# pvangoor/eqvio

Hardware: AMD Instinct MI355X
Metric: EqF vision updates/sec @ N=200 landmarks (higher is better)
Workload: dtype f64; 1 GPU; synthetic 'hover' world, 200 tracked landmarks (state dim 621, 400 measurement rows), InvDepth chart, fast Riccati, IMU 200 Hz / camera 20 Hz (10 observer steps per frame), EuRoC pinhole intrinsics, one independent filter per GPU (replicas); landmarks=200, state_dim=621, parallelism=replicas x1

## Files before the change

eqvio_amd/csrc/eqf_kernels.hpp:

```cpp
#pragma once
#include "eqf_math.hpp"
#include "eqvio_types.h"
#include <hip/hip_runtime.h>

namespace eqf {

struct Common {
    double Mv[9];
    double RTic[9];
    double RTicSx[9];
    double CT[36];
    double vC[3];
    double Ass[441];
    double Bs[252];
};
struct CommonK {
    double lm[66];
    double RA[9];
    double SxRA[9];
    double RAsv[9];
    double G[9];
    double adT[36];
};
constexpr int kObsChunk = 20;
struct RiccatiArgs {
    double dt;
    double Qd[12];
    double Pd[8];
};
struct ObsStep {
    int discrete;
    double dt;
    Pose Tinv;
    V3 omC, vC;
};

__device__ __forceinline__ V3 ld3(const double* base, int stride, int i) { return V3{base[i], base[stride + i], base[2 * stride + i]}; }
__device__ __forceinline__ Qt ldq(const double* base, int stride, int i) { return Qt{base[i], base[stride + i], base[2 * stride + i], base[3 * stride + i]}; }
__device__ __forceinline__ M3 ldm3(const double* p) { return M3{p[0], p[1], p[2], p[3], p[4], p[5], p[6], p[7], p[8]}; }
__device__ __forceinline__ void st_plane9(double* base, int stride, int i, int plane0, const M3& A) {
    base[(plane0 + 0) * stride + i] = A.a00;
    base[(plane0 + 1) * stride + i] = A.a01;
    base[(plane0 + 2) * stride + i] = A.a02;
    base[(plane0 + 3) * stride + i] = A.a10;
    base[(plane0 + 4) * stride + i] = A.a11;
    base[(plane0 + 5) * stride + i] = A.a12;
    base[(plane0 + 6) * stride + i] = A.a20;
    base[(plane0 + 7) * stride + i] = A.a21;
    base[(plane0 + 8) * stride + i] = A.a22;
}

typedef unsigned long long trace_t;
__device__ __forceinline__ void trace_start(trace_t* tr) {
    if (tr && blockIdx.x == 0 && blockIdx.y == 0 && threadIdx.x == 0)
        *tr = wall_clock64();
}
__device__ __forceinline__ void trace_end(trace_t* tr) {
    if (tr && threadIdx.x == 0)
        atomicMax(tr + 1, (trace_t)wall_clock64());
}

__device__ __forceinline__ double fast_rcp(double d) {
    double r = __builtin_amdgcn_rcp(d);
    double e = fma(-d, r, 1.0);
    r = fma(r, e, r);
    e = fma(-d, r, 1.0);
    return fma(r, e, r);
}

__device__ __forceinline__ double fast_rsqrt(double x) {
    double y = __builtin_amdgcn_rsq(x);
    double h = 0.5 * x;
    y = y * fma(-h * y, y, 1.5);
    y = y * fma(-h * y, y, 1.5);
    return y;
}
constexpr int CC_OFF = 3, CC_E2I = 0, CC_I2E = 9, CC_R0 = 18, CC_PLANES = 27;
__device__ __forceinline__ M3 ld_cc(const double* __restrict__ q0, int Ncap, int i, int which) {
    const double* b = q0 + (size_t)(CC_OFF + which) * Ncap + i;
    return M3{b[0], b[Ncap], b[2 * (size_t)Ncap], b[3 * (size_t)Ncap], b[4 * (size_t)Ncap], b[5 * (size_t)Ncap], b[6 * (size_t)Ncap], b[7 * (size_t)Ncap], b[8 * (size_t)Ncap]};
}
__device__ __attribute__((noinline)) void store_chart_constants(double* __restrict__ cc, int Ncap, int i, double px, double py, double pz, M3* r0) {
    const V3 p{px, py, pz};
    st_plane9(cc, Ncap, i, CC_E2I, conv_euc2ind(p));
    st_plane9(cc, Ncap, i, CC_I2E, conv_ind2euc(p));
    const M3 R = ind2euc_r0(p);
    st_plane9(cc, Ncap, i, CC_R0, R);
    if (r0)
        *r0 = R;
}

__host__ __device__ __forceinline__ int al_col(int e) { return e < 3 ? e : (e < 6 ? 12 + (e - 3) : 15 + (e - 6)); }

__device__ __forceinline__ double sensor_Bs_entry(const CommonK& ck, int t) {
    const int r = t / 12, c = t % 12;
    double v = 0.0;
    if (r < 6)
        v = (c == 6 + r) ? 1.0 : 0.0;
    else if (r < 9 && c < 3)
        v = ck.RA[(r - 6) * 3 + c];
    else if (r >= 9 && r < 12 && c < 3)
        v = ck.SxRA[(r - 9) * 3 + c];
    else if (r >= 12 && r < 15 && c < 3)
        v = ck.RAsv[(r - 12) * 3 + c];
    else if (r >= 12 && r < 15 && c >= 3 && c < 6)
        v = ck.RA[(r - 12) * 3 + (c - 3)];
    return v;
}
__device__ __forceinline__ double sensor_Ass_entry(const CommonK& ck, int t) {
    const int r = t / 21, c = t % 21;
    double v = 0.0;
    if (c < 6) {
        if (r >= 6 && r < 9 && c < 3)
            v = -ck.RA[(r - 6) * 3 + c];
        else if (r >= 9 && r < 12 && c < 3)
            v = -ck.SxRA[(r - 9) * 3 + c];
        else if (r >= 12 && r < 15 && c < 3)
            v = -ck.RAsv[(r - 12) * 3 + c];
        else if (r >= 12 && r < 15 && c >= 3)
            v = -ck.RA[(r - 12) * 3 + (c - 3)];
    } else if (r >= 9 && r < 12 && c == r + 3) {
        v = 1.0;
    } else if (r >= 12 && r < 15 && c >= 6 && c < 9) {
        v = ck.G[(r - 12) * 3 + (c - 6)];
    } else if (r >= 15 && c >= 15) {
        v = ck.adT[(r - 15) * 6 + (c - 15)];
    }
    return v;
}
template <int PART>
__device__ __forceinline__ void assemble_landmark(const double* __restrict__ s_cm, int chart, const V3 p0, const Qt q, const double a, const M3& e2i, const M3& i2e,
                                                  double (&al)[45], double (&bl)[9]) {
    constexpr bool P0 = PART < 0 || PART == 0, P1 = PART < 0 || PART == 1, P2 = PART < 0 || PART == 2;
    const M3 Mv = ldm3(s_cm), RTic = ldm3(s_cm + 9), RTicSx = ldm3(s_cm + 18);
    const double* CT = s_cm + 27;
    const V3 vC{s_cm[63], s_cm[64], s_cm[65]};
    const M3 RQ = q_mat(q);
    const M3 Qhat = a * RQ;
    const V3 qh = (1.0 / a) * (transpose(RQ) * p0);
    const bool ind = chart == EQVIO_COORD_INVDEPTH;
    if (P0) {
        M3 Bblk = Qhat * (skew(qh) * RTic + RTicSx);
        M3 A_v = (-1.0) * (Qhat * Mv);
        if (ind) {
            Bblk = e2i * Bblk;
            A_v = e2i * A_v;
        }
        const M3 A_b = (-1.0) * Bblk;
        const double ab[9] = {A_b.a00, A_b.a01, A_b.a02, A_b.a10, A_b.a11, A_b.a12, A_b.a20, A_b.a21, A_b.a22};
        const double av[9] = {A_v.a00, A_v.a01, A_v.a02, A_v.a10, A_v.a11, A_v.a12, A_v.a20, A_v.a21, A_v.a22};
#pragma unroll
        for (int r = 0; r < 3; ++r)
#pragma unroll
            for (int c = 0; c < 3; ++c) {
                al[r * 15 + c] = ab[r * 3 + c];
                al[r * 15 + 3 + c] = av[r * 3 + c];
            }
        bl[0] = Bblk.a00, bl[1] = Bblk.a01, bl[2] = Bblk.a02, bl[3] = Bblk.a10, bl[4] = Bblk.a11, bl[5] = Bblk.a12, bl[6] = Bblk.a20, bl[7] = Bblk.a21, bl[8] = Bblk.a22;
    }
    if (P1) {
        const M3 T0 = skew(p0) * RQ;
        const M3 T1 = (-a) * RQ;
        const double t[3][6] = {{T0.a00, T0.a01, T0.a02, T1.a00, T1.a01, T1.a02},
                                {T0.a10, T0.a11, T0.a12, T1.a10, T1.a11, T1.a12},
                                {T0.a20, T0.a21, T0.a22, T1.a20, T1.a21, T1.a22}};
        double Ac[3][6];
#pragma unroll
        for (int r = 0; r < 3; ++r)
#pragma unroll
            for (int c = 0; c < 6; ++c) {
                double s = 0;
#pragma unroll
                for (int k = 0; k < 6; ++k)
                    s += t[r][k] * CT[k * 6 + c];
                Ac[r][c] = s;
            }
        if (ind) {
            const double e[3][3] = {{e2i.a00, e2i.a01, e2i.a02}, {e2i.a10, e2i.a11, e2i.a12}, {e2i.a20, e2i.a21, e2i.a22}};
            double Ac2[3][6];
#pragma unroll
            for (int r = 0; r < 3; ++r)
#pragma unroll
                for (int c = 0; c < 6; ++c)
                    Ac2[r][c] = e[r][0] * Ac[0][c] + e[r][1] * Ac[1][c] + e[r][2] * Ac[2][c];
#pragma unroll
            for (int r = 0; r < 3; ++r)
#pragma unroll
                for (int c = 0; c < 6; ++c)
                    Ac[r][c] = Ac2[r][c];
        }
#pragma unroll
        for (int r = 0; r < 3; ++r)
#pragma unroll
            for (int c = 0; c < 6; ++c)
                al[r * 15 + 6 + c] = Ac[r][c];
    }
    if (P2) {
        const M3 inner = skew(qh) * skew(vC) - 2.0 * outer(vC, qh) + outer(qh, vC);
        const M3 QhatInv = (1.0 / a) * transpose(RQ);
        M3 A_q = (-1.0 / norm2(qh)) * (Qhat * inner * QhatInv);
        if (ind)
            A_q = e2i * A_q * i2e;
        const double aq[9] = {A_q.a00, A_q.a01, A_q.a02, A_q.a10, A_q.a11, A_q.a12, A_q.a20, A_q.a21, A_q.a22};
#pragma unroll
        for (int r = 0; r < 3; ++r)
#pragma unroll
            for (int c = 0; c < 3; ++c)
                al[r * 15 + 12 + c] = aq[r * 3 + c];
    }
}
__global__ void __launch_bounds__(64) k_assemble_AB(const CommonK ck, int N, int Ncap, int chart, Common* __restrict__ cmdev,
                                                    const double* __restrict__ q0, const double* __restrict__ Qq, const double* __restrict__ Qa,
                                                    double* __restrict__ Al, double* __restrict__ Bl, trace_t* tr) {
    trace_start(tr);
    __shared__ double s_cm[9 + 9 + 9 + 36 + 3];
    for (int t = threadIdx.x; t < 66; t += blockDim.x)
        s_cm[t] = ck.lm[t];
    {
        const int gt = blockIdx.x * blockDim.x + threadIdx.x, gs = gridDim.x * blockDim.x;
        for (int t = gt; t < 252; t += gs)
            cmdev->Bs[t] = sensor_Bs_entry(ck, t);
        for (int t = gt; t < 441; t += gs)
            cmdev->Ass[t] = sensor_Ass_entry(ck, t);
    }
    __syncthreads();
    const int i = blockIdx.x * blockDim.x + threadIdx.x;
    if (i >= N)
        return;
    double al[45], bl[9];
    const bool ind = chart == EQVIO_COORD_INVDEPTH;
    assemble_landmark<-1>(s_cm, chart, ld3(q0, Ncap, i), ldq(Qq, Ncap, i), Qa[i], ind ? ld_cc(q0, Ncap, i, CC_E2I) : M3{}, ind ? ld_cc(q0, Ncap, i, CC_I2E) : M3{}, al, bl);
#pragma unroll
    for (int e = 0; e < 45; ++e)
        Al[e * Ncap + i] = al[e];
#pragma unroll
    for (int e = 0; e < 9; ++e)
        Bl[e * Ncap + i] = bl[e];
}

struct ObsSteps {
    ObsStep s[kObsChunk];
};
__device__ __forceinline__ void observer_chain(const ObsStep* __restrict__ steps, int k, const V3 p0, Qt& q, double& a) {
    double inva = 1.0 / a;
    ObsStep nxt = steps[0];
    for (int s = 0; s < k; ++s) {
        const ObsStep st = nxt;
        nxt = steps[min(s + 1, k - 1)];
        const V3 ph = inva * q_rot(q_inv(q), p0);
        Qt Lq;
        double La, invLa;
        if (st.discrete) {
            const V3 p1 = pose_act(st.Tinv, ph);
            const double nh2 = norm2(ph), n12 = norm2(p1);
            const double r = fast_rsqrt(nh2 * n12);
            const double c = dot(p1, ph) * r;
            if (c < -1.0 + 1e-12) {
                Lq = so3_from_vectors(normalized(p1), normalized(ph));
            } else {
                const V3 ax = r * cross(p1, ph);
                const double t = (1.0 + c) * 2.0;
                const double is = fast_rsqrt(t);
                const Qt L{0.5 * (t * is), ax.x * is, ax.y * is, ax.z * is};
                const double kk = 1.5 - 0.5 * (L.w * L.w + L.x * L.x + L.y * L.y + L.z * L.z);
                Lq = Qt{L.w * kk, L.x * kk, L.y * kk, L.z * kk};
            }
            La = nh2 * r;
            invLa = n12 * r;
        } else {
            const double ip2 = 1.0 / norm2(ph);
            const V3 Wr = st.omC + ip2 * cross(ph, st.vC);
            const double Ws = ip2 * dot(ph, st.vC);
            Lq = so3_exp(st.dt * Wr);
            La = exp(st.dt * Ws);
            invLa = 1.0 / La;
        }
        if (st.discrete) {
            const Qt m{q.w * Lq.w - q.x * Lq.x - q.y * Lq.y - q.z * Lq.z, q.w * Lq.x + q.x * Lq.w + q.y * Lq.z - q.z * Lq.y,
                       q.w * Lq.y + q.y * Lq.w + q.z * Lq.x - q.x * Lq.z, q.w * Lq.z + q.z * Lq.w + q.x * Lq.y - q.y * Lq.x};
            const double km = 1.5 - 0.5 * (m.w * m.w + m.x * m.x + m.y * m.y + m.z * m.z);
            q = Qt{m.w * km, m.x * km, m.y * km, m.z * km};
// ... 1114 lines not shown
            swork[tid] = z;
        }
        __syncthreads();
        const int wr = i0 + tid - m;
        if (tid < 32 && wr >= 0 && wr < rows - 1 - m) {
            double gsum = 0.0;
            for (int c = 0; c < w; ++c)
                gsum = fma(sPI[tid + c * CH_LDP], swork[c], gsum);
            gpart[(size_t)GAMMA_G * ldg + wr] = gsum;
        }
    }
    if (!update)
        return;
    const bool next_diag = (blockIdx.x == 0 && blockIdx.y == 0);
    {
        const double* pj = diag_tile ? sPI : sPJ;
        d4 acc = {0, 0, 0, 0};
#pragma unroll
        for (int st = 0; st < 8; ++st) {
            const int c = 4 * st + lk;
            const double a = sPI[16 * ihU + lr + c * CH_LDP];
            const double b = pj[16 * jhU + lr + c * CH_LDP];
            acc = __builtin_amdgcn_mfma_f64_16x16x4f64(b, a, acc, 0, 0, 0);
        }
        const int i = i0 + 16 * ihU + lr;
#pragma unroll
        for (int q = 0; q < 4; ++q) {
            const int j = j0 + 16 * jhU + lk + 4 * q;
            const double v = zt[q] - acc[q];
            if (i < rows && j < m && (!next_diag || i >= m))
                Z[i + (size_t)j * ldz] = v;
            if (next_diag)
                sPJ[16 * ihU + lr + (16 * jhU + lk + 4 * q) * CH_LDP] = v;
        }
    }
    if (!next_diag)
        return;
    __syncthreads();
    const int w2 = min(32, m - c0);
#pragma unroll
    for (int k = 0; k < 4; ++k) {
        const int c = g + 8 * k;
        if (r >= w2 || c >= w2)
            sPJ[r + c * CH_LDP] = (r == c) ? 1.0 : 0.0;
    }
    __syncthreads();
    ldl_inverse_tile(sPJ, CH_LDP, w2, LinvOut, flags, swork);
}

template <typename TS, bool FUSED, bool SYM = false, bool GH = false>
__global__ void __launch_bounds__(PROP_T) k_propagate_main(int N, int Ncap, int ld, RiccatiArgs ra, const Common* __restrict__ cm,
                                                        const TS* __restrict__ Sig, TS* __restrict__ Sout, const double* __restrict__ Al,
                                                        const double* __restrict__ Bl, int nT, int tpw, const ObsSteps obs, int obs_k,
                                                        const double* __restrict__ q0, double* __restrict__ Qq, double* __restrict__ Qa, int nObs, const StageArgs sg,
                                                        trace_t* tr, const FuseArgs fa, const MeasEval me, const GatherArgs ga_in) {
    GatherArgs ga;
    if constexpr (GH)
        ga = ga_in;
    else {
        ga.n = 0, ga.nprop = N, ga.held = nullptr, ga.st_in = nullptr, ga.st_out = nullptr;
    }
    trace_start(tr);
    const double dt = ra.dt;
    const int b = blockIdx.x;
    const int tid = threadIdx.x;
    constexpr bool sym = SYM;
    constexpr int nStrip = 0;
    int nTiles = sym ? nT * (nT + 1) / 2 : nT * nT;
    if (sym && tpw > 1) {
        nTiles = 0;
        for (int r_ = 0; r_ < nT; ++r_)
            nTiles += (r_ + tpw) / tpw;
    }
    __shared__ double sm[2 * PT * (63 + 36 + 9 + 9) + 63 * PT + 12 * 21 + 8];
    __shared__ double sJ1[PT * (63 + 36 + 9 + 9)];
    if (b > nTiles + nStrip + nObs) {
        for (int t = tid; t < 2 * sg.M; t += PROP_T)
            sg.y_d[t] = sg.y_h[t];
        for (int t = tid; t < sg.M; t += PROP_T)
            sg.idx_d[t] = sg.idx_h[t];
        for (int t = tid; t < 3 * N; t += PROP_T) {
            const int pl = t / N, i = t - pl * N;
            sg.ylm_d[pl * Ncap + i] = sg.ylm_h[pl * Ncap + i];
        }
        return;
    }
    if (b > nTiles + nStrip) {
        const int i = (b - (nTiles + nStrip + 1)) * PROP_T + tid;
        static_assert(sizeof(ObsStep) % 8 == 0 && kObsChunk * sizeof(ObsStep) <= sizeof(sm), "the steps are copied as doubles into the tile buffer");
        if (FUSED) {
            for (int t = tid; t < obs_k * (int)(sizeof(ObsStep) / 8); t += PROP_T)
                sm[t] = reinterpret_cast<const double*>(obs.s)[t];
            __syncthreads();
        }
        const ObsStep* steps_lds = reinterpret_cast<const ObsStep*>(sm);
        if (i < N) {
            if (FUSED) {
                const bool held = i >= ga.nprop;
                const bool synth = held && ga.held != nullptr;
                const int io = held ? i : gather_old(ga, i);
                V3 p0;
                Qt q;
                double a_;
                if (synth) {
                    const double* hp = ga.held + 1 + 3 * (i - ga.nprop);
                    p0 = V3{hp[0], hp[1], hp[2]};
                    q = Qt{1.0, 0.0, 0.0, 0.0};
                    a_ = 1.0;
                } else {
                    p0 = ld3(q0, Ncap, io);
                    q = ldq(Qq, Ncap, io);
                    a_ = Qa[io];
                }
                double yu = 0.0, yv = 0.0;
                int jm = -1;
                if (me.on) {
                    yu = me.ylm[i], yv = me.ylm[Ncap + i];
                    jm = (int)me.ylm[2 * Ncap + i];
                }
                M3 r0_new{};
                if (synth) {
                    double* st = ga.st_out;
                    st[i] = p0.x;
                    st[Ncap + i] = p0.y;
                    st[2 * (size_t)Ncap + i] = p0.z;
                    double* cc = st + (size_t)CC_OFF * Ncap;
                    store_chart_constants(cc, Ncap, i, p0.x, p0.y, p0.z, &r0_new);
                }
                if (!held)
                    observer_chain(steps_lds, obs_k, p0, q, a_);
                fa.Qqo[i] = q.w;
                fa.Qqo[Ncap + i] = q.x;
                fa.Qqo[2 * Ncap + i] = q.y;
                fa.Qqo[3 * Ncap + i] = q.z;
                fa.Qao[i] = a_;
                if (me.on && jm >= 0) {
                    asm volatile("" : "+v"(q.w), "+v"(q.x), "+v"(q.y), "+v"(q.z), "+v"(a_));
                    const MeasOut o = measure_one(fa.chart, me.cam, p0, q, a_, yu, yv, me.star != 0, fa.chart == EQVIO_COORD_INVDEPTH ? (synth ? r0_new : ld_cc(q0, Ncap, io, CC_R0)) : M3{});
#pragma unroll
                    for (int e = 0; e < 6; ++e)
                        me.C[e * me.Mcap + jm] = o.c[e];
                    me.ytil[2 * jm] = o.yt[0];
                    me.ytil[2 * jm + 1] = o.yt[1];
                    me.lmidx_dev[jm] = i;
                }
            } else {
                observer_landmark(obs.s, Ncap, obs_k, i, q0, Qq, Qa, Qq, Qa);
            }
        }
        return;
    }
    __shared__ double sSens[21 * 33];
    __shared__ double sSens1[21 * 33];
    __shared__ double s_cm[66];
    if (FUSED) {
        for (int t = tid; t < 66; t += PROP_T)
            s_cm[t] = fa.ck.lm[t];
        __syncthreads();
    }
    if (b < nTiles) {
        int bi = b % nT, bj0 = b / nT, ntile = 1;
        if (sym && tpw > 1) {
            int base = 0;
            bi = 0;
            for (;;) {
                const int w_ = (bi + tpw) / tpw;
                if (b < base + w_)
                    break;
                base += w_;
                ++bi;
            }
            bj0 = (b - base) * tpw;
            ntile = min(tpw, bi + 1 - bj0);
        } else if (sym) {
            bi = (int)((sqrtf(8.0f * (float)b + 1.0f) - 1.0f) * 0.5f);
            while (bi * (bi + 1) / 2 > b)
                --bi;
            while ((bi + 1) * (bi + 2) / 2 <= b)
                ++bi;
            bj0 = b - bi * (bi + 1) / 2;
        }
        const int nb = sym ? bi + 1 : nT;
        const int Nprop = FUSED ? ga.nprop : N;
        const int Nmem = (FUSED && ga.held) ? Nprop : N;
        const double held_var = (FUSED && ga.held && Nprop < N) ? ga.held[0] : 0.0;
        double* sGi = sm;
        double* sFi = sGi + 63 * PT;
        double* sDi = sFi + 36 * PT;
        double* sBi = sDi + 9 * PT;
        double* sJ0 = sBi + 9 * PT;
        double* sSi = sJ0 + 117 * PT;
        double* sSs = sSi + 63 * PT;
        const int r = tid / (PT * PT), tp = tid % (PT * PT);
        const int ti = tp % PT, tj = tp / PT;
        auto stage = [&](const int it) {
            const bool first = it == 0;
            const int bj = bj0 + it;
            double* sSj = (it & 1) ? sJ1 : sJ0;
            double* sFj = sSj + 63 * PT;
            double* sDj = sFj + 36 * PT;
            double* sBj = sDj + 9 * PT;
            double* sSn = (it & 1) ? sSens1 : sSens;
            for (int t = tid; t < 63 * PT; t += PROP_T) {
                const int e = t / PT, x = t % PT;
                const int i = bi * PT + x, j = bj * PT + x;
                const int kk = e / 3, cc = e % 3;
                if (first)
                    sSi[t] = i < Nmem ? Sig[kk + (size_t)(21 + 3 * (i < Nprop ? gather_old(ga, i) : i) + cc) * ld] : 0.0;
                sSj[t] = j < Nmem ? Sig[kk + (size_t)(21 + 3 * (j < Nprop ? gather_old(ga, j) : j) + cc) * ld] : 0.0;
            }
            if (first && tid < 12 * 21)
                sSs[tid] = Sig[al_col(tid / 21) + (size_t)(tid % 21) * ld];
            const int ncol = bj < 21 ? (21 - bj + nb - 1) / nb : 0;
            for (int t = PROP_T - 1 - tid; t < ncol * 33; t += PROP_T) {
                const int m_ = t / 33, e = t % 33;
                const int c = bj + nb * m_;
                sSn[t] = e < 21 ? (FUSED ? sensor_Ass_entry(fa.ck, c * 21 + e) : cm->Ass[c * 21 + e]) : (FUSED ? sensor_Bs_entry(fa.ck, c * 12 + (e - 21)) : cm->Bs[c * 12 + (e - 21)]);
            }
            if (FUSED) {
                const int part = tid >> 6, lane_ = tid & 63;
                if (part < 3 && lane_ < 2 * PT && (first || lane_ >= PT)) {
                    const bool isj = lane_ >= PT;
                    const int x = lane_ % PT;
                    const int l = (isj ? bj : bi) * PT + x;
                    double* dF = isj ? sFj : sFi;
                    double* dD = isj ? sDj : sDi;
                    double* dB = isj ? sBj : sBi;
                    double al[45], bl[9];
#pragma unroll
                    for (int e = 0; e < 45; ++e)
                        al[e] = 0.0;
#pragma unroll
                    for (int e = 0; e < 9; ++e)
                        bl[e] = 0.0;
                    const bool in = l < Nprop;
                    const bool heldl = l >= Nprop && l < N;
                    const bool ind = fa.chart == EQVIO_COORD_INVDEPTH;
                    const int lc = in ? gather_old(ga, l) : 0;
                    const V3 p0_ = ld3(q0, Ncap, lc);
                    const Qt q_ = ldq(Qq, Ncap, lc);
                    const double a_ = Qa[lc];
                    const M3 e2i = ind ? ld_cc(q0, Ncap, lc, CC_E2I) : M3{};
                    if (part == 0) {
                        if (in)
                            assemble_landmark<0>(s_cm, fa.chart, p0_, q_, a_, e2i, M3{}, al, bl);
#pragma unroll
                        for (int rr = 0; rr < 3; ++rr) {
#pragma unroll
                            for (int c = 0; c < 6; ++c)
                                dF[(rr * 12 + c) * PT + x] = in ? dt * al[rr * 15 + c] : 0.0;
#pragma unroll
                            for (int c = 0; c < 3; ++c)
                                dB[(rr * 3 + c) * PT + x] = bl[rr * 3 + c];
                        }
                    } else if (part == 1) {
                        if (in)
                            assemble_landmark<1>(s_cm, fa.chart, p0_, q_, a_, e2i, M3{}, al, bl);
#pragma unroll
                        for (int rr = 0; rr < 3; ++rr)
#pragma unroll
                            for (int c = 6; c < 12; ++c)
                                dF[(rr * 12 + c) * PT + x] = in ? dt * al[rr * 15 + c] : 0.0;
                    } else {
                        if (in)
                            assemble_landmark<2>(s_cm, fa.chart, p0_, q_, a_, e2i, ind ? ld_cc(q0, Ncap, lc, CC_I2E) : M3{}, al, bl);
#pragma unroll
                        for (int rr = 0; rr < 3; ++rr)
#pragma unroll
                            for (int c = 0; c < 3; ++c)
                                dD[(rr * 3 + c) * PT + x] = in ? dt * al[rr * 15 + 12 + c] + ((rr == c) ? 1.0 : 0.0) : ((heldl && rr == c) ? 1.0 : 0.0);
                    }
                }
            } else {
                for (int t = tid; t < 36 * PT; t += PROP_T) {
                    const int e = t / PT, x = t % PT;
                    const int rr = e / 12, c = e % 12;
                    const int i = bi * PT + x, j = bj * PT + x;
                    if (first)
                        sFi[t] = i < N ? dt * Al[(rr * 15 + c) * Ncap + i] : 0.0;
                    sFj[t] = j < N ? dt * Al[(rr * 15 + c) * Ncap + j] : 0.0;
                }
                for (int t = tid; t < 9 * PT; t += PROP_T) {
                    const int e = t / PT, x = t % PT;
                    const int rr = e / 3, c = e % 3;
                    const int i = bi * PT + x, j = bj * PT + x;
                    const double eye = (rr == c) ? 1.0 : 0.0;
                    if (first) {
                        sDi[t] = i < N ? dt * Al[(rr * 15 + 12 + c) * Ncap + i] + eye : 0.0;
                        sBi[t] = i < N ? Bl[e * Ncap + i] : 0.0;
                    }
                    sDj[t] = j < N ? dt * Al[(rr * 15 + 12 + c) * Ncap + j] + eye : 0.0;
                    sBj[t] = j < N ? Bl[e * Ncap + j] : 0.0;
                }
            }
        };
        stage(0);
        __syncthreads();
        for (int t = tid; t < 63 * PT; t += PROP_T) {
            const int e = t / PT, x = t % PT;
            const int rr = e / 21, k = e % 21;
            double g = 0.0;
#pragma unroll
            for (int q = 0; q < 12; ++q)
                g += sFi[(rr * 12 + q) * PT + x] * sSs[q * 21 + k];
#pragma unroll
            for (int cc = 0; cc < 3; ++cc)
                g += sDi[(rr * 3 + cc) * PT + x] * sSi[(k * 3 + cc) * PT + x];
            sGi[t] = g;
        }
        __syncthreads();
        for (int it = 0; it < ntile; ++it) {
            const int bj = bj0 + it;
            const double* sSj = (it & 1) ? sJ1 : sJ0;
            const double* sFj = sSj + 63 * PT;
            const double* sDj = sFj + 36 * PT;
            const double* sBj = sDj + 9 * PT;
            const double* sSn = (it & 1) ? sSens1 : sSens;
            const int ncol = bj < 21 ? (21 - bj + nb - 1) / nb : 0;
            const int i = bi * PT + ti, j = bj * PT + tj;
            const bool mine = !(i >= N || j >= N || (sym && bi == bj && i < j));
            const int li = 21 + 3 * i, lj = 21 + 3 * j;
            double Sij[3][3];
            if (mine) {
                if (i < Nmem && j < Nmem) {
                    const int lio = 21 + 3 * (i < Nprop ? gather_old(ga, i) : i), ljo = 21 + 3 * (j < Nprop ? gather_old(ga, j) : j);
#pragma unroll
                    for (int k = 0; k < 3; ++k)
#pragma unroll
                        for (int c = 0; c < 3; ++c)
                            Sij[k][c] = Sig[lio + k + (size_t)(ljo + c) * ld];
                } else {
#pragma unroll
                    for (int k = 0; k < 3; ++k)
#pragma unroll
                        for (int c = 0; c < 3; ++c)
                            Sij[k][c] = (i == j && k == c) ? held_var : 0.0;
                }
            }
            if (it + 1 < ntile)
                stage(it + 1);
            {
                for (int t = tid; t < PT * 3 * ncol; t += PROP_T) {
                    const int x = t % PT, rc = t / PT;
                    const int rr = rc % 3, m_ = rc / 3, c = bj + nb * m_;
                    const int ii = bi * PT + x;
                    if (ii < N) {
                        double sacc = 0;
                        for (int k = 0; k < 21; ++k) {
                            const double f = dt * sSn[m_ * 33 + k] + (k == c ? 1.0 : 0.0);
                            sacc += sGi[(rr * 21 + k) * PT + x] * f;
                        }
                        double bq = 0;
#pragma unroll
                        for (int q = 0; q < 3; ++q)
                            bq += sBi[(rr * 3 + q) * PT + x] * ra.Qd[q] * sSn[m_ * 33 + 21 + q];
                        sacc += dt * bq;
                        const int lii = 21 + 3 * ii;
                        Sout[lii + rr + (size_t)c * ld] = sacc;
                        Sout[c + (size_t)(lii + rr) * ld] = sacc;
                    }
                }
            }
            if (mine) {
                double E[3];
#pragma unroll
                for (int c = 0; c < 3; ++c) {
                    double s = 0;
#pragma unroll
                    for (int e = 0; e < 12; ++e)
                        s += sFi[(r * 12 + e) * PT + ti] * sSj[(al_col(e) * 3 + c) * PT + tj];
#pragma unroll
                    for (int k = 0; k < 3; ++k)
                        s += sDi[(r * 3 + k) * PT + ti] * Sij[k][c];
                    E[c] = s;
                }
#pragma unroll
                for (int c = 0; c < 3; ++c) {
                    double s = 0;
#pragma unroll
                    for (int e = 0; e < 12; ++e)
                        s += sGi[(r * 21 + al_col(e)) * PT + ti] * sFj[(c * 12 + e) * PT + tj];
#pragma unroll
                    for (int k = 0; k < 3; ++k)
                        s += E[k] * sDj[(c * 3 + k) * PT + tj];
                    double bq = 0;
#pragma unroll
                    for (int q = 0; q < 3; ++q)
                        bq += sBi[(r * 3 + q) * PT + ti] * ra.Qd[q] * sBj[(c * 3 + q) * PT + tj];
                    s += dt * bq;
                    if (i == j && r == c && i < Nprop)
                        s += dt * ra.Pd[7];
                    Sout[li + r + (size_t)(lj + c) * ld] = s;
                    if (sym && i != j)
                        Sout[lj + c + (size_t)(li + r) * ld] = s;
                }
            }
            if (it + 1 < ntile)
                __syncthreads();
        }
        return;
    }
    {
        if (FUSED && ga.n) {
            const int Np = ga.nprop;
            for (int t = tid; t < (CC_OFF + CC_PLANES) * Np; t += PROP_T) {
                const int pl = t / Np, i = t - pl * Np;
                ga.st_out[(size_t)pl * Ncap + i] = ga.st_in[(size_t)pl * Ncap + gather_old(ga, i)];
            }
        }
        double* sF = sm;
        double* sS = sm + 441;
        double* sT = sm + 882;
        double* sBs = sm + 1323;
        for (int t = tid; t < 441; t += PROP_T) {
            const int r = t / 21, c = t % 21;
            sF[t] = dt * (FUSED ? sensor_Ass_entry(fa.ck, t) : cm->Ass[t]) + (r == c ? 1.0 : 0.0);
            sS[t] = Sig[r + (size_t)c * ld];
        }
        for (int t = tid; t < 252; t += PROP_T)
            sBs[t] = FUSED ? sensor_Bs_entry(fa.ck, t) : cm->Bs[t];
        __syncthreads();
        for (int t = tid; t < 441; t += PROP_T) {
            const int r = t / 21, c = t % 21;
            double s = 0;
            for (int k = 0; k < 21; ++k)
                s += sF[r * 21 + k] * sS[k * 21 + c];
            sT[t] = s;
        }
        __syncthreads();
        for (int t = tid; t < 441; t += PROP_T) {
            const int r = t / 21, c = t % 21;
            double s = 0;
            for (int k = 0; k < 21; ++k)
                s += sT[r * 21 + k] * sF[c * 21 + k];
            double bq = 0;
            for (int q = 0; q < 12; ++q)
                bq += sBs[r * 12 + q] * ra.Qd[q] * sBs[c * 12 + q];
            s += dt * bq;
            if (r == c)
                s += dt * ra.Pd[r / 3];
            Sout[r + (size_t)c * ld] = s;
        }
    }
}


#ifndef EQF_SYRK_UNROLL
#define EQF_SYRK_UNROLL 4
#endif
struct TileRed {
    double v[4];
};
template <bool WITH_GEMV, int NW = 4>
__device__ __forceinline__ TileRed mfma_tile32_splitk(const double* __restrict__ P, int ldp, int i0, int rowsP, const double* __restrict__ Qm, int ldq, int j0,
                                                      int rowsQ, int K, double* __restrict__ sred , const double* __restrict__ zvec = nullptr,
                                                      int ldzv = 0, double* gv_out = nullptr) {
    const int tid = threadIdx.x;
    const int wave = tid >> 6, lane = tid & 63;
    const int lr = lane & 15, lk = lane >> 4;
    const int ia = min(i0 + lr, rowsP - 1), ib = min(i0 + 16 + lr, rowsP - 1);
    const int ja = min(j0 + lr, rowsQ - 1), jb = min(j0 + 16 + lr, rowsQ - 1);
    const double zia = (i0 + lr < rowsP) ? 1.0 : 0.0, zib = (i0 + 16 + lr < rowsP) ? 1.0 : 0.0;
    const double zja = (j0 + lr < rowsQ) ? 1.0 : 0.0, zjb = (j0 + 16 + lr < rowsQ) ? 1.0 : 0.0;
    d4 acc00 = {0, 0, 0, 0}, acc10 = acc00, acc01 = acc00, acc11 = acc00;
    double ga = 0.0, gb = 0.0;
    const int nsteps = (K + 3) >> 2;
#pragma unroll EQF_SYRK_UNROLL
    for (int st = wave; st < nsteps; st += NW) {
        const int kk = 4 * st + lk;
        const int kc = min(kk, K - 1);
        const double zk = kk < K ? 1.0 : 0.0;
        const double pa = P[ia + (size_t)kc * ldp] * (zia * zk);
        const double pb = P[ib + (size_t)kc * ldp] * (zib * zk);
        const double qa = Qm[ja + (size_t)kc * ldq] * zja;
        const double qb = Qm[jb + (size_t)kc * ldq] * zjb;
        if (WITH_GEMV) {
            const double zv = zvec[(size_t)kc * ldzv];
            ga = fma(pa, zv, ga);
            gb = fma(pb, zv, gb);
        }
        acc00 = __builtin_amdgcn_mfma_f64_16x16x4f64(qa, pa, acc00, 0, 0, 0);
        acc10 = __builtin_amdgcn_mfma_f64_16x16x4f64(qa, pb, acc10, 0, 0, 0);
        acc01 = __builtin_amdgcn_mfma_f64_16x16x4f64(qb, pa, acc01, 0, 0, 0);
        acc11 = __builtin_amdgcn_mfma_f64_16x16x4f64(qb, pb, acc11, 0, 0, 0);
    }
    TileRed out;
#pragma unroll
    for (int e = 0; e < 4; ++e)
        out.v[e] = 0.0;
#pragma unroll
    for (int q0 = 0; q0 < NW; q0 += 4) {
        if (q0)
            __syncthreads();
        if (wave >= q0 && wave < q0 + 4) {
            double* mine = sred + (wave - q0) * 1024;
#pragma unroll
            for (int r = 0; r < 4; ++r) {
                const int j = lk + 4 * r;
                mine[lr + 32 * j] = acc00[r];
                mine[16 + lr + 32 * j] = acc10[r];
                mine[lr + 32 * (16 + j)] = acc01[r];
                mine[16 + lr + 32 * (16 + j)] = acc11[r];
            }
        }
        __syncthreads();
#pragma unroll
        for (int e = 0; e < 4; ++e) {
            const int idx = (tid & 31) + 32 * (((tid & 255) >> 5) + 8 * e);
            out.v[e] += (sred[idx] + sred[1024 + idx]) + (sred[2048 + idx] + sred[3072 + idx]);
        }
    }
    if (WITH_GEMV) {
        __syncthreads();
        sred[(wave * 4 + lk) * 32 + lr] = ga;
        sred[(wave * 4 + lk) * 32 + 16 + lr] = gb;
        __syncthreads();
        if (tid < 32) {
            double g = 0.0;
#pragma unroll
            for (int q = 0; q < 4 * NW; ++q)
                g += sred[q * 32 + tid];
            *gv_out = g;
        }
    }
    return out;
}

__global__ void __launch_bounds__(256) k_gamma(int n, int m, int ldz, const double* __restrict__ Wb, double* __restrict__ gamma) {
    __shared__ double sp[256];
    const int r = blockIdx.x * 64 + (threadIdx.x & 63);
    const int seg = threadIdx.x >> 6;
    const double* W = Wb + m;
    const double* z = Wb + m + n;
    double s0 = 0, s1 = 0, s2 = 0, s3 = 0;
    if (r < n) {
        int p = seg;
        for (; p + 12 < m; p += 16) {
            s0 += W[r + (size_t)p * ldz] * z[(size_t)p * ldz];
            s1 += W[r + (size_t)(p + 4) * ldz] * z[(size_t)(p + 4) * ldz];
            s2 += W[r + (size_t)(p + 8) * ldz] * z[(size_t)(p + 8) * ldz];
            s3 += W[r + (size_t)(p + 12) * ldz] * z[(size_t)(p + 12) * ldz];
        }
        for (; p < m; p += 4)
            s0 += W[r + (size_t)p * ldz] * z[(size_t)p * ldz];
    }
    sp[threadIdx.x] = (s0 + s1) + (s2 + s3);
    __syncthreads();
    if (seg == 0 && r < n)
        gamma[r] = (sp[threadIdx.x] + sp[64 + threadIdx.x]) + (sp[128 + threadIdx.x] + sp[192 + threadIdx.x]);
}

constexpr int SYRK_ARITH_TILES = 24;
constexpr int SYRK_NW = 8;
template <typename TS, bool WITH_GAMMA>
__device__ __forceinline__ void syrk_sub_tile(int n, int m, int ld, int ldz, const double* __restrict__ Wb, TS* __restrict__ Sig, double* __restrict__ gamma, const int* __restrict__ spec,
                                              int spec_seq, const int* __restrict__ flags, trace_t* tr, const int* __restrict__ tile_of_block, int stall_seq, int blk, const int* __restrict__ live_cols = nullptr, int nt_arith = 0) {
    if (tr && blk == 0 && threadIdx.x == 0)
        *tr = wall_clock64();
    const int f0 = flags[0], f3 = flags[3];
    const int specv = spec ? *spec : 0;
    __shared__ double sred[1024 * 4];
    int bi, bj;
    if (nt_arith > 0) {
        bi = (int)((sqrtf(8.0f * (float)blk + 1.0f) - 1.0f) * 0.5f);
        while ((bi + 1) * (bi + 2) / 2 <= blk)
            ++bi;
        while (bi * (bi + 1) / 2 > blk)
            --bi;
        bj = blk - bi * (bi + 1) / 2;
    } else {
        const int code = tile_of_block[blk];
        bi = code & 0xffff, bj = code >> 16;
    }
// ... 968 lines not shown
```

Baseline: 11590 updates/s.

## Split propagate tile staging across warps and stage sensor constants in LDS

In the fused covariance propagation kernel, warps 0-2 now issue their landmark-state loads early, while the remaining threads batch-load the Sigma landmark/sensor blocks into registers before writing them to shared memory. The whole CommonK struct is also copied into LDS, and the sensor Ass/Bs entries are read from there with index-based lookups instead of branchy reads from kernel arguments. The goal is to overlap global-load latency with assembly work and cut repeated constant-parameter reads. In exchange the code carries more complex thread-role logic, extra registers for the batched loads, and a changed synchronisation pattern.

```diff
diff --git a/eqvio_amd/csrc/eqf_kernels.hpp b/eqvio_amd/csrc/eqf_kernels.hpp
--- a/eqvio_amd/csrc/eqf_kernels.hpp
+++ b/eqvio_amd/csrc/eqf_kernels.hpp
@@ -127,6 +127,36 @@
         v = ck.adT[(r - 15) * 6 + (c - 15)];
     }
     return v;
+}
+constexpr int CK_RA = 66, CK_G = CK_RA + 27, CK_ADT = CK_G + 9, CK_DOUBLES = CK_ADT + 36;
+static_assert(sizeof(CommonK) == CK_DOUBLES * sizeof(double), "CommonK is read as doubles");
+__device__ __forceinline__ double sensor_Bs_entry_lds(const double* s_ck, int t) {
+    const int r = t / 12, c = t % 12, blk = r / 3;
+    int idx = -1;
+    if (blk >= 2 && blk <= 4 && c < 3)
+        idx = CK_RA + 9 * (blk - 2) + (r - 3 * blk) * 3 + c;
+    else if (blk == 4 && c < 6)
+        idx = CK_RA + (r - 12) * 3 + (c - 3);
+    const double v = s_ck[max(idx, 0)];
+    return idx >= 0 ? v : ((r < 6 && c == 6 + r) ? 1.0 : 0.0);
+}
+__device__ __forceinline__ double sensor_Ass_entry_lds(const double* s_ck, int t) {
+    const int r = t / 21, c = t % 21, blk = r / 3;
+    int idx = -1;
+    bool neg = false;
+    if (c < 6) {
+        neg = true;
+        if (blk >= 2 && blk <= 4 && c < 3)
+            idx = CK_RA + 9 * (blk - 2) + (r - 3 * blk) * 3 + c;
+        else if (blk == 4)
+            idx = CK_RA + (r - 12) * 3 + (c - 3);
+    } else if (blk == 4 && c < 9) {
+        idx = CK_G + (r - 12) * 3 + (c - 6);
+    } else if (r >= 15 && c >= 15) {
+        idx = CK_ADT + (r - 15) * 6 + (c - 15);
+    }
+    const double v = s_ck[max(idx, 0)];
+    return idx >= 0 ? (neg ? -v : v) : ((blk == 3 && c == r + 3) ? 1.0 : 0.0);
 }
 template <int PART>
 __device__ __forceinline__ void assemble_landmark(const double* __restrict__ s_cm, int chart, const V3 p0, const Qt q, const double a, const M3& e2i, const M3& i2e,
@@ -1547,10 +1577,11 @@
     }
     __shared__ double sSens[21 * 33];
     __shared__ double sSens1[21 * 33];
-    __shared__ double s_cm[66];
-    if (FUSED) {
-        for (int t = tid; t < 66; t += PROP_T)
-            s_cm[t] = fa.ck.lm[t];
+    __shared__ double s_ck[CK_DOUBLES];
+    const double* const s_cm = s_ck;
+    if (FUSED && b >= nTiles) {
+        for (int t = tid; t < CK_DOUBLES; t += PROP_T)
+            s_ck[t] = reinterpret_cast<const double*>(&fa.ck)[t];
         __syncthreads();
     }
     if (b < nTiles) {
@@ -1596,28 +1627,113 @@
             double* sDj = sFj + 36 * PT;
             double* sBj = sDj + 9 * PT;
             double* sSn = (it & 1) ? sSens1 : sSens;
-            for (int t = tid; t < 63 * PT; t += PROP_T) {
-                const int e = t / PT, x = t % PT;
-                const int i = bi * PT + x, j = bj * PT + x;
-                const int kk = e / 3, cc = e % 3;
-                if (first)
-                    sSi[t] = i < Nmem ? Sig[kk + (size_t)(21 + 3 * (i < Nprop ? gather_old(ga, i) : i) + cc) * ld] : 0.0;
-                sSj[t] = j < Nmem ? Sig[kk + (size_t)(21 + 3 * (j < Nprop ? gather_old(ga, j) : j) + cc) * ld] : 0.0;
-            }
-            if (first && tid < 12 * 21)
-                sSs[tid] = Sig[al_col(tid / 21) + (size_t)(tid % 21) * ld];
             const int ncol = bj < 21 ? (21 - bj + nb - 1) / nb : 0;
-            for (int t = PROP_T - 1 - tid; t < ncol * 33; t += PROP_T) {
-                const int m_ = t / 33, e = t % 33;
-                const int c = bj + nb * m_;
-                sSn[t] = e < 21 ? (FUSED ? sensor_Ass_entry(fa.ck, c * 21 + e) : cm->Ass[c * 21 + e]) : (FUSED ? sensor_Bs_entry(fa.ck, c * 12 + (e - 21)) : cm->Bs[c * 12 + (e - 21)]);
+            if (!FUSED) {
+                for (int t = tid; t < 63 * PT; t += PROP_T) {
+                    const int e = t / PT, x = t % PT;
+                    const int i = bi * PT + x, j = bj * PT + x;
+                    const int kk = e / 3, cc = e % 3;
+                    if (first)
+                        sSi[t] = i < N ? Sig[kk + (size_t)(21 + 3 * i + cc) * ld] : 0.0;
+                    sSj[t] = j < N ? Sig[kk + (size_t)(21 + 3 * j + cc) * ld] : 0.0;
+                }
+                if (first && tid < 12 * 21)
+                    sSs[tid] = Sig[al_col(tid / 21) + (size_t)(tid % 21) * ld];
+                for (int t = PROP_T - 1 - tid; t < ncol * 33; t += PROP_T) {
+                    const int m_ = t / 33, e = t % 33;
+                    const int c = bj + nb * m_;
+                    sSn[t] = e < 21 ? cm->Ass[c * 21 + e] : cm->Bs[c * 12 + (e - 21)];
+                }
             }
             if (FUSED) {
+                constexpr int NA = 3 * 64, NC = PROP_T - NA, SIJ = 63 * PT, NK = (2 * SIJ + 12 * 21 + NC - 1) / NC;
                 const int part = tid >> 6, lane_ = tid & 63;
-                if (part < 3 && lane_ < 2 * PT && (first || lane_ >= PT)) {
-                    const bool isj = lane_ >= PT;
-                    const int x = lane_ % PT;
-                    const int l = (isj ? bj : bi) * PT + x;
+                const bool assembles = part < 3 && lane_ < 2 * PT && (first || lane_ >= PT);
+                const bool isj = lane_ >= PT;
+                const int x = lane_ % PT;
+                const int l = (isj ? bj : bi) * PT + x;
+                const bool in = l < Nprop;
+                const bool heldl = l >= Nprop && l < N;
+                const bool ind = fa.chart == EQVIO_COORD_INVDEPTH;
+                V3 p0_{};
+                Qt q_{};
+                double a_ = 0.0;
+                M3 e2i{}, i2e{};
+                auto request_state = [&]() {
+                    if (assembles) {
+                        const int lc = in ? gather_old(ga, l) : 0;
+                        p0_ = ld3(q0, Ncap, lc);
+                        q_ = ldq(Qq, Ncap, lc);
+                        a_ = Qa[lc];
+                        if (ind)
+                            e2i = ld_cc(q0, Ncap, lc, CC_E2I);
+                        if (ind && part == 2)
+                            i2e = ld_cc(q0, Ncap, lc, CC_I2E);
+                    }
+                };
+                if (first)
+                    request_state();
+                if (tid >= NA) {
+                    const int u = tid - NA;
+                    constexpr int TOT = 2 * SIJ + 12 * 21;
+                    auto item = [&](const int t, size_t& off, bool& inmem) -> double* {
+                        const bool ss = t >= 2 * SIJ, js = t >= SIJ && !ss;
+                        const int s_ = t - (ss ? 2 * SIJ : (js ? SIJ : 0));
+                        const int kk = s_ % 21, ci = s_ / 21, xs = ci / 3, cc = ci % 3;
+                        const int ls = (js ? bj : bi) * PT + xs;
+                        inmem = ss || ls < Nmem;
+                        const size_t off_l = kk + (size_t)(21 + 3 * (ls < Nprop ? gather_old(ga, ls) : ls) + cc) * ld;
+                        const int e12 = s_ % 12, k21 = s_ / 12;
+                        const size_t off_s = al_col(e12) + (size_t)k21 * ld;
+                        off = inmem ? (ss ? off_s : off_l) : 0;
+                        return ss ? sSs + e12 * 21 + k21 : (js ? sSj : sSi) + (kk * 3 + cc) * PT + xs;
+                    };
+                    if (first) {
+                        static_assert(NK * NC - TOT <= NC && NK * NC >= TOT, "the lanes past the end take an item of the row above once more");
+                        double v[NK];
+                        double ckv = reinterpret_cast<const double*>(&fa.ck)[min(u, CK_DOUBLES - 1)];
+#pragma unroll
+                        for (int k = 0; k < NK; ++k) {
+                            const int t = u + k * NC;
+                            size_t off;
+                            bool inmem;
+                            item(t < TOT ? t : t - NC, off, inmem);
+                            const double sv = Sig[off];
+                            v[k] = inmem ? sv : 0.0;
+                        }
+                        asm volatile("" : "+v"(ckv));
+#pragma unroll
+                        for (int k = 0; k < NK; ++k) {
+                            const int t = u + k * NC;
+                            size_t off;
+                            bool inmem;
+                            *item(t < TOT ? t : t - NC, off, inmem) = v[k];
+                        }
+                        if (u < CK_DOUBLES)
+                            s_ck[u] = ckv;
+                    } else {
+#pragma unroll 1
+                        for (int t = SIJ + u; t < 2 * SIJ; t += NC) {
+                            size_t off;
+                            bool inmem;
+                            double* dst = item(t, off, inmem);
+                            const double sv = Sig[off];
+                            *dst = inmem ? sv : 0.0;
+                        }
+                    }
+                }
+                if (first)
+                    __syncthreads();
+                else
+                    request_state();
+                if (tid >= NA) {
+                    for (int t = tid - NA; t < ncol * 33; t += NC) {
+                        const int m_ = t / 33, e = t % 33;
+                        const int c = bj + nb * m_;
+                        sSn[t] = e < 21 ? sensor_Ass_entry_lds(s_ck, c * 21 + e) : sensor_Bs_entry_lds(s_ck, c * 12 + (e - 21));
+                    }
+                }
+                if (assembles) {
                     double* dF = isj ? sFj : sFi;
                     double* dD = isj ? sDj : sDi;
                     double* dB = isj ? sBj : sBi;
@@ -1628,14 +1744,9 @@
 #pragma unroll
                     for (int e = 0; e < 9; ++e)
                         bl[e] = 0.0;
-                    const bool in = l < Nprop;
-                    const bool heldl = l >= Nprop && l < N;
-                    const bool ind = fa.chart == EQVIO_COORD_INVDEPTH;
-                    const int lc = in ? gather_old(ga, l) : 0;
-                    const V3 p0_ = ld3(q0, Ncap, lc);
-                    const Qt q_ = ldq(Qq, Ncap, lc);
-                    const double a_ = Qa[lc];
-                    const M3 e2i = ind ? ld_cc(q0, Ncap, lc, CC_E2I) : M3{};
+                    asm volatile("" : "+v"(p0_.x), "+v"(p0_.y), "+v"(p0_.z), "+v"(q_.w), "+v"(q_.x), "+v"(q_.y), "+v"(q_.z), "+v"(a_));
+                    asm volatile("" : "+v"(e2i.a00), "+v"(e2i.a01), "+v"(e2i.a02), "+v"(e2i.a10), "+v"(e2i.a11), "+v"(e2i.a12), "+v"(e2i.a20), "+v"(e2i.a21), "+v"(e2i.a22));
+                    asm volatile("" : "+v"(i2e.a00), "+v"(i2e.a01), "+v"(i2e.a02), "+v"(i2e.a10), "+v"(i2e.a11), "+v"(i2e.a12), "+v"(i2e.a20), "+v"(i2e.a21), "+v"(i2e.a22));
                     if (part == 0) {
                         if (in)
                             assemble_landmark<0>(s_cm, fa.chart, p0_, q_, a_, e2i, M3{}, al, bl);
@@ -1658,7 +1769,7 @@
                                 dF[(rr * 12 + c) * PT + x] = in ? dt * al[rr * 15 + c] : 0.0;
                     } else {
                         if (in)
-                            assemble_landmark<2>(s_cm, fa.chart, p0_, q_, a_, e2i, ind ? ld_cc(q0, Ncap, lc, CC_I2E) : M3{}, al, bl);
+                            assemble_landmark<2>(s_cm, fa.chart, p0_, q_, a_, e2i, i2e, al, bl);
 #pragma unroll
                         for (int rr = 0; rr < 3; ++rr)
 #pragma unroll
@@ -1809,11 +1920,11 @@
         double* sBs = sm + 1323;
         for (int t = tid; t < 441; t += PROP_T) {
             const int r = t / 21, c = t % 21;
-            sF[t] = dt * (FUSED ? sensor_Ass_entry(fa.ck, t) : cm->Ass[t]) + (r == c ? 1.0 : 0.0);
+            sF[t] = dt * (FUSED ? sensor_Ass_entry_lds(s_ck, t) : cm->Ass[t]) + (r == c ? 1.0 : 0.0);
             sS[t] = Sig[r + (size_t)c * ld];
         }
         for (int t = tid; t < 252; t += PROP_T)
-            sBs[t] = FUSED ? sensor_Bs_entry(fa.ck, t) : cm->Bs[t];
+            sBs[t] = FUSED ? sensor_Bs_entry_lds(s_ck, t) : cm->Bs[t];
         __syncthreads();
         for (int t = tid; t < 441; t += PROP_T) {
             const int r = t / 21, c = t % 21;
```

Result: no change. 11560 updates/s, median of 2 (-0.2%).
